# KRLabsOrg/verbatim-rag

Measured on AMD Instinct MI355X. Metric: query x chunk span-extractions/sec @512tok (ModernBERT-base extractor, chunks/s), higher is better.
Workload: dtype bf16

## Files before the change

verbatim-rag_amd/csrc/qkv_attn.hip:

```cpp
#include "host_util.h"
#include "qkv_attn.h"

#include <algorithm>
#include <cstdlib>
#include <type_traits>
#include <vector>

#ifdef VRAG_DEBUG_API
#define VRAG_DBG(bit) ((p.debug_flags & (bit)) != 0)
#else
#define VRAG_DBG(bit) false
#endif

namespace vrag {

constexpr int QA_WB = 192 * 128;
constexpr int QA_XOFF = 2 * QA_WB;
constexpr int QA_TAB = 131072;
constexpr int QA_MU = QA_TAB, QA_RS = QA_TAB + 2048, QA_LS = QA_TAB + 4096;
constexpr int QA_CA = QA_TAB + 5120, QA_SA = QA_CA + 4096, QA_CB = QA_SA + 4096, QA_SB = QA_CB + 2048;
constexpr int QA_SMEM = QA_SB + 2048;
constexpr int QA_V_OFF = 65536;

constexpr float QA_LAZY = 8.0f;
__device__ __forceinline__ float max3f(float a, float b, float c) { return __builtin_fmaxf(__builtin_fmaxf(a, b), c); }

template <int N>
__device__ __forceinline__ void wait_vm() {
  asm volatile("s_waitcnt vmcnt(%0)" ::"n"(N) : "memory");
}

template <bool LOCAL, bool FOLD, typename T>
__global__ __launch_bounds__(512, 2) void qkv_attn_kernel(const QkvAttnParams p) {
  typedef typename Op<T>::v4 V4;
  typedef typename Op<T>::v8 V8;
  extern __shared__ __attribute__((aligned(16))) char smem[];
  const int tid = threadIdx.x;
  const int lane = tid & 63;
  const int wave = uniform(tid >> 6);
  const int g = lane >> 4, l15 = lane & 15;
  const int H = p.H, Tp = p.Tp, nh = p.nh;
  const int xcd = blockIdx.x & 7, slot = blockIdx.x >> 3;
  const int grp = (slot / nh) * 8 + xcd, head = slot % nh;
  if (grp >= p.n_groups) return;
  const int4 wd = p.groups[grp * 8 + wave];
  const int wrow0 = uniform(wd.x), S = uniform(wd.y), kbase = uniform(wd.z);
  const int srow0 = wave * 64;
  const int qrow0 = (wave - kbase) * 64;
  const bool active = qrow0 < S;
  const T* X = reinterpret_cast<const T*>(p.x);
  const T* Wh = reinterpret_cast<const T*>(p.w) + (size_t)head * 192 * H;

  unsigned voffX[2], voffW[3];
#pragma unroll
  for (int par = 0; par < 2; ++par) {
    const int r = par * 8 + (lane >> 3);
    voffX[par] = (unsigned)(r * H + (((lane & 7) ^ ((r >> 1) & 7)) << 3)) * 2u;
  }
#pragma unroll
  for (int i = 0; i < 3; ++i) {
    const int row = wave * 24 + i * 8 + (lane >> 3);
    voffW[i] = (unsigned)(row * H + (((lane & 7) ^ ((row >> 1) & 7)) << 3)) * 2u;
  }
  const char* const Xw = reinterpret_cast<const char*>(X + (size_t)wrow0 * H);
  const char* const Wb = reinterpret_cast<const char*>(Wh);
  char* const xbuf = smem + QA_XOFF + wave * 8192;
  auto dma_w = [&](int kt, int buf, int i) {
    if (VRAG_DBG(4)) return;
    unsigned vo = voffW[i];
    asm volatile("" : "+v"(vo));
    glds16(Wb + kt * 128 + vo, smem + buf * QA_WB + (wave * 24 + i * 8) * 128);
  };
  auto dma_x = [&](int kt, int i) {
    if (!active || VRAG_DBG(4)) return;
    unsigned vo = voffX[i & 1];
    asm volatile("" : "+v"(vo));
    glds16(Xw + ((size_t)(i >> 1) * 16 * H + kt * 64) * 2 + vo, xbuf + i * 1024);
  };

  if (!VRAG_DBG(4)) {
    if (FOLD && lane < 16) {
      glds16(p.ln_mu + min(wrow0 + lane * 4, Tp - 4), smem + QA_MU + srow0 * 4);
      glds16(p.ln_rstd + min(wrow0 + lane * 4, Tp - 4), smem + QA_RS + srow0 * 4);
    }
    if (FOLD && wave == 2) glds16(p.ln_s + head * 192 + lane * 4, smem + QA_LS);
    if (wave == 2 || wave == 3) {
      const float* tab = wave == 2 ? p.rope_cos : p.rope_sin;
#pragma unroll
      for (int i = 0; i < 2; ++i) {
        const int r = i * 8 + (lane >> 3);
        glds16(tab + min(r, p.rope_rows - 1) * 32 + (((lane & 7) ^ ((r >> 1) & 7)) << 2), smem + (wave == 2 ? QA_CB : QA_SB) + i * 1024);
      }
    }
    if (wave == 4 || wave == 5) {
      const float* tab = wave == 4 ? p.rope_cos : p.rope_sin;
#pragma unroll
      for (int i = 0; i < 4; ++i)
        glds16(tab + (size_t)min(16 * (i * 8 + (lane >> 3)), p.rope_rows - 1) * 32 + (lane & 7) * 4, smem + (wave == 4 ? QA_CA : QA_SA) + i * 1024);
    }
  }

  f32x4 acc[12][4];
#pragma unroll
  for (int a = 0; a < 12; ++a)
#pragma unroll
    for (int c = 0; c < 4; ++c) acc[a][c] = f32x4{0.f, 0.f, 0.f, 0.f};

  const int KT = H >> 6;
  int fo[2];
#pragma unroll
  for (int s2 = 0; s2 < 2; ++s2) fo[s2] = l15 * 128 + ((((4 * s2 + g) ^ ((l15 >> 1) & 7))) << 4);
#ifdef VRAG_DEBUG_API
  const int probe = p.debug_flags;
#else
  int probe = 0;
  asm volatile("" : "+s"(probe));
#endif
  const bool mm = active && !(probe & 2);
#pragma unroll
  for (int i = 0; i < 3; ++i) dma_w(0, 0, i);
#pragma unroll
  for (int i = 0; i < 8; ++i) dma_x(0, i);
  for (int kt = 0; kt < KT; ++kt) {
    wait_vm<0>();
    __builtin_amdgcn_s_barrier();
    asm volatile("" ::: "memory");
    const char* sW = smem + (kt & 1) * QA_WB;
    const bool more = kt + 1 < KT;
    V8 xf[2][4], wa;
    if (mm) {
#pragma unroll
      for (int s2 = 0; s2 < 2; ++s2)
#pragma unroll
        for (int rt = 0; rt < 4; ++rt) xf[s2][rt] = *reinterpret_cast<const V8*>(xbuf + rt * 16 * 128 + fo[s2]);
      wa = *reinterpret_cast<const V8*>(sW + fo[0]);
    }
    asm volatile("s_waitcnt lgkmcnt(0)" ::: "memory");
    __builtin_amdgcn_sched_barrier(0);
    if (mm) {
#pragma unroll
      for (int it = 0; it < 24; ++it) {
        const int s2 = it / 12, nj = it % 12;
        V8 na = wa;
        if (it < 23) na = *reinterpret_cast<const V8*>(sW + ((it + 1) % 12) * 16 * 128 + fo[(it + 1) / 12]);
        __builtin_amdgcn_sched_barrier(0);
#pragma unroll
        for (int rt = 0; rt < 4; ++rt) {
          if (nj < 8) acc[nj][rt] = Op<T>::mfma16(wa, xf[s2][rt], acc[nj][rt]);
          else acc[nj][rt] = Op<T>::mfma16(xf[s2][rt], wa, acc[nj][rt]);
        }
        __builtin_amdgcn_sched_barrier(0);
        if (more && it < 11) {
          if (it < 3) dma_w(kt + 1, (kt + 1) & 1, it);
          else dma_x(kt + 1, it - 3);
        }
        __builtin_amdgcn_sched_barrier(0);
        wa = na;
      }
    } else if (more) {
#pragma unroll
      for (int i = 0; i < 3; ++i) dma_w(kt + 1, (kt + 1) & 1, i);
#pragma unroll
      for (int i = 0; i < 8; ++i) dma_x(kt + 1, i);
    }
  }
  __syncthreads();
  if (VRAG_DBG(16)) return;

  const float* l_mu = reinterpret_cast<const float*>(smem + QA_MU) + srow0;
  const float* l_rs = reinterpret_cast<const float*>(smem + QA_RS) + srow0;
  const float* l_ls = reinterpret_cast<const float*>(smem + QA_LS);
#pragma unroll
  for (int db = 0; db < 4; ++db) {
    const int d = db * 16 + l15;
    const float lsv = FOLD ? l_ls[128 + d] : 0.f;
#pragma unroll
    for (int tp = 0; tp < 2; ++tp) {
      V8 vv;
#pragma unroll
      for (int a = 0; a < 2; ++a) {
        const int rt = 2 * tp + a;
        f32x4 m4 = {0.f, 0.f, 0.f, 0.f}, r4 = {1.f, 1.f, 1.f, 1.f};
        if constexpr (FOLD) {
          m4 = *reinterpret_cast<const f32x4*>(l_mu + rt * 16 + 4 * g);
          r4 = *reinterpret_cast<const f32x4*>(l_rs + rt * 16 + 4 * g);
        }
#pragma unroll
        for (int h = 0; h < 2; ++h) {
          const int r0 = 2 * h;
          const f32x2 v = pk_fma(f32x2{-m4[r0], -m4[r0 + 1]}, splat2(lsv), f32x2{acc[8 + db][rt][r0], acc[8 + db][rt][r0 + 1]}) * f32x2{r4[r0], r4[r0 + 1]};
#pragma unroll
          for (int e = 0; e < 2; ++e)
            vv[a * 4 + r0 + e] = qrow0 + rt * 16 + 4 * g + r0 + e < S ? Op<T>::to(v[e], p.f16_sat) : (T)0.f;
        }
      }
      const int c = wave * 8 + tp * 4 + g;
      *reinterpret_cast<V8*>(smem + QA_V_OFF + d * 1024 + ((c ^ l15) << 4)) = vv;
    }
  }
  auto rope_rows = [&](int a0, int rt, int ls_off, float scale, V8 (&out)[2]) {
    const bool live = qrow0 + rt * 16 + l15 < S;
    const float mu = FOLD ? l_mu[rt * 16 + l15] : 0.f, rs = FOLD ? l_rs[rt * 16 + l15] : 1.f;
#pragma unroll
    for (int np = 0; np < 2; ++np) {
      const int dd = np * 16 + 4 * g;
      const f32x4 ca = *reinterpret_cast<const f32x4*>(smem + QA_CA + (((qrow0 >> 4) + rt) * 32 + dd) * 4);
      const f32x4 sa = *reinterpret_cast<const f32x4*>(smem + QA_SA + (((qrow0 >> 4) + rt) * 32 + dd) * 4);
      const int bsw = l15 * 128 + ((((dd >> 2) ^ ((l15 >> 1) & 7))) << 4);
      const f32x4 cb = *reinterpret_cast<const f32x4*>(smem + QA_CB + bsw);
      const f32x4 sb = *reinterpret_cast<const f32x4*>(smem + QA_SB + bsw);
      f32x4 l1 = {0.f, 0.f, 0.f, 0.f}, l2 = {0.f, 0.f, 0.f, 0.f};
      if constexpr (FOLD) {
        l1 = *reinterpret_cast<const f32x4*>(l_ls + ls_off + dd);
        l2 = *reinterpret_cast<const f32x4*>(l_ls + ls_off + 32 + dd);
      }
#pragma unroll
      for (int h = 0; h < 2; ++h) {
        const int j0 = 2 * h;
        f32x2 x1 = {acc[a0 + np][rt][j0], acc[a0 + np][rt][j0 + 1]}, x2 = {acc[a0 + 2 + np][rt][j0], acc[a0 + 2 + np][rt][j0 + 1]};
        if constexpr (FOLD) {
          x1 = pk_fma(splat2(-mu), f32x2{l1[j0], l1[j0 + 1]}, x1) * rs;
          x2 = pk_fma(splat2(-mu), f32x2{l2[j0], l2[j0 + 1]}, x2) * rs;
        }
        const f32x2 ca2 = {ca[j0], ca[j0 + 1]}, sa2 = {sa[j0], sa[j0 + 1]}, cb2 = {cb[j0], cb[j0 + 1]}, sb2 = {sb[j0], sb[j0 + 1]};
        const f32x2 c = pk_fma(-sa2, sb2, ca2 * cb2), sn = pk_fma(ca2, sb2, sa2 * cb2);
        const f32x2 o1 = pk_fma(-x2, sn, x1 * c) * scale, o2 = pk_fma(x1, sn, x2 * c) * scale;
#pragma unroll
        for (int e = 0; e < 2; ++e) {
          if constexpr (!std::is_same<T, bf16_t>::value) {
            out[0][np * 4 + j0 + e] = live ? Op<T>::to(o1[e], p.f16_sat) : (T)0.f;
            out[1][np * 4 + j0 + e] = live ? Op<T>::to(o2[e], p.f16_sat) : (T)0.f;
          } else {
            out[0][np * 4 + j0 + e] = Op<T>::to(o1[e], p.f16_sat);
            out[1][np * 4 + j0 + e] = Op<T>::to(o2[e], p.f16_sat);
          }
        }
      }
    }
  };
#pragma unroll
  for (int rt = 0; rt < 4; ++rt) {
    V8 kf[2];
    rope_rows(4, rt, 64, 1.0f, kf);
    const int row = srow0 + rt * 16 + l15;
#pragma unroll
    for (int s = 0; s < 2; ++s) *reinterpret_cast<V8*>(smem + row * 128 + (((4 * s + g) ^ ((row >> 1) & 7)) << 4)) = kf[s];
  }
  V8 qf[4][2];
#pragma unroll
  for (int rt = 0; rt < 4; ++rt) rope_rows(0, rt, 0, p.q_scale, qf[rt]);
  __syncthreads();

  f32x4 ot[4][4];
  f32x4 lo[4];
#pragma unroll
  for (int c = 0; c < 4; ++c) {
    lo[c] = f32x4{0.f, 0.f, 0.f, 0.f};
#pragma unroll
    for (int dt = 0; dt < 4; ++dt) ot[c][dt] = f32x4{0.f, 0.f, 0.f, 0.f};
  }
  float m_run[4] = {0.f, 0.f, 0.f, 0.f};
  bool seen[4] = {false, false, false, false};
  V8 ones;
#pragma unroll
  for (int j = 0; j < 8; ++j) ones[j] = (T)1.0f;
  const int W = p.window;
  int kt_lo = 0, kt_hi = (S - 1) >> 6;
  if constexpr (LOCAL) {
    kt_lo = max(0, qrow0 - W) >> 6;
    kt_hi = min(S - 1, qrow0 + 63 + W) >> 6;
  }
  const int ksw = (l15 >> 1) & 7;
  if (active && !VRAG_DBG(1)) {
    for (int kt = kt_lo; kt <= kt_hi; ++kt) {
      bool cut[2][2];
#pragma unroll
      for (int u = 0; u < 2; ++u) {
        const int q_lo = qrow0 + 32 * u;
#pragma unroll
        for (int t2 = 0; t2 < 2; ++t2) {
          const int kh = kt * 64 + t2 * 32;
          bool outside = kh >= S || q_lo >= S;
          cut[u][t2] = kh + 31 >= S;
          if constexpr (LOCAL) {
            outside = outside || (kh + 31 < q_lo - W) || (kh > q_lo + 31 + W);
            cut[u][t2] = cut[u][t2] || (kh < q_lo + 31 - W) || (kh + 31 > q_lo + W);
          }
          cut[u][t2] = cut[u][t2] || outside;
        }
      }
      V8 pf[4][2];
      {
        f32x4 st[4][4];
#pragma unroll
        for (int c = 0; c < 4; ++c) {
          const float seed = -m_run[c];
#pragma unroll
          for (int kb = 0; kb < 4; ++kb) st[c][kb] = f32x4{seed, seed, seed, seed};
        }
#pragma unroll
        for (int kb = 0; kb < 4; ++kb) {
          const char* krow = smem + ((kbase + kt) * 64 + kb * 16 + l15) * 128;
          const V8 k0 = *reinterpret_cast<const V8*>(krow + ((g ^ ksw) << 4));
          const V8 k1 = *reinterpret_cast<const V8*>(krow + (((4 + g) ^ ksw) << 4));
#pragma unroll
          for (int c = 0; c < 4; ++c) {
            st[c][kb] = Op<T>::mfma16(k0, qf[c][0], st[c][kb]);
            st[c][kb] = Op<T>::mfma16(k1, qf[c][1], st[c][kb]);
          }
        }
        float mx[4];
#pragma unroll
        for (int c = 0; c < 4; ++c) {
          const int u = c >> 1;
          mx[c] = -INFINITY;
#pragma unroll
          for (int t2 = 0; t2 < 2; ++t2) {
            if (cut[u][t2]) {
              const int qi = qrow0 + 16 * c + l15;
              int lo_k = 0, hi_k = S - 1;
              if constexpr (LOCAL) {
                lo_k = max(0, qi - W);
                hi_k = min(S - 1, qi + W);
              }
              const unsigned span = hi_k >= lo_k ? (unsigned)(hi_k - lo_k) : 0u;
              int d0 = hi_k >= lo_k ? kt * 64 + t2 * 32 + 4 * g - lo_k : -100000;
              asm volatile("" : "+v"(d0));
#pragma unroll
              for (int h2 = 0; h2 < 2; ++h2)
#pragma unroll
                for (int r = 0; r < 4; ++r) {
                  const bool ok = (unsigned)(d0 + 16 * h2 + r) <= span;
                  st[c][2 * t2 + h2][r] = ok ? st[c][2 * t2 + h2][r] : -INFINITY;
                }
            }
            const f32x4& a = st[c][2 * t2];
            const f32x4& b2 = st[c][2 * t2 + 1];
            mx[c] = max3f(mx[c], max3f(a[0], a[1], a[2]), max3f(a[3], b2[0], b2[1]));
            mx[c] = max3f(mx[c], b2[2], b2[3]);
          }
        }
        bool move = false;
#pragma unroll
        for (int c = 0; c < 4; ++c) {
          const bool qlive = qrow0 + 16 * c + l15 < S;
          move = move || (qlive && (mx[c] > QA_LAZY || (!seen[c] && mx[c] > -INFINITY)));
        }
        if (__any(move)) {
#pragma unroll
          for (int c = 0; c < 4; ++c) {
            float m_all = fmaxf(mx[c], __shfl_xor(mx[c], 16, 64));
            m_all = fmaxf(m_all, __shfl_xor(m_all, 32, 64));
            const bool has = m_all > -INFINITY;
            const float delta = seen[c] ? fmaxf(m_all, 0.f) : (has ? m_all : 0.f);
            const float alpha = seen[c] ? __builtin_amdgcn_exp2f(-delta) : 1.0f;
            seen[c] = seen[c] || has;
            m_run[c] += delta;
#pragma unroll
            for (int kb = 0; kb < 4; ++kb)
#pragma unroll
              for (int r = 0; r < 4; ++r) st[c][kb][r] -= delta;
#pragma unroll
            for (int dt = 0; dt < 4; ++dt)
#pragma unroll
              for (int r = 0; r < 4; ++r) ot[c][dt][r] *= alpha;
#pragma unroll
            for (int r = 0; r < 4; ++r) lo[c][r] *= alpha;
          }
        }
#pragma unroll
        for (int c = 0; c < 4; ++c)
#pragma unroll
          for (int t2 = 0; t2 < 2; ++t2)
#pragma unroll
            for (int j = 0; j < 8; ++j) pf[c][t2][j] = (T)__builtin_amdgcn_exp2f(st[c][2 * t2 + (j >> 2)][j & 3]);
      }
#pragma unroll
      for (int t2 = 0; t2 < 2; ++t2) {
#pragma unroll
        for (int c = 0; c < 4; ++c) lo[c] = Op<T>::mfma16(ones, pf[c][t2], lo[c]);
#pragma unroll
        for (int dt = 0; dt < 4; ++dt) {
          const V8 vf = *reinterpret_cast<const V8*>(smem + QA_V_OFF + (dt * 16 + l15) * 1024 + ((((kbase + kt) * 8 + t2 * 4 + g) ^ l15) << 4));
#pragma unroll
          for (int c = 0; c < 4; ++c) ot[c][dt] = Op<T>::mfma16(vf, pf[c][t2], ot[c][dt]);
        }
      }
    }
  }
  __syncthreads();

  if (active) {
    char* stg = smem + wave * 8192;
#pragma unroll
    for (int rt = 0; rt < 4; ++rt) {
      const int row = rt * 16 + l15;
      const bool live = qrow0 + row < S;
      const float inv = live ? 1.0f / lo[rt][0] : 0.f;
#pragma unroll
      for (int db = 0; db < 4; ++db) {
        V4 o;
#pragma unroll
        for (int j = 0; j < 4; ++j) o[j] = live ? Op<T>::to(ot[rt][db][j] * inv, p.f16_sat) : (T)0.f;
        const int c16 = db * 2 + (g >> 1);
        *reinterpret_cast<V4*>(stg + row * 128 + ((c16 ^ (row & 7)) << 4) + ((g & 1) << 3)) = o;
      }
    }
#pragma unroll
    for (int it = 0; it < 8; ++it) {
      const int row = it * 8 + (lane >> 3), c16 = lane & 7;
      const f32x4 v = *reinterpret_cast<const f32x4*>(stg + row * 128 + ((c16 ^ (row & 7)) << 4));
      if (qrow0 + row < S && !VRAG_DBG(8)) store16_nt(reinterpret_cast<T*>(p.o) + (size_t)(wrow0 + row) * H + head * 64 + c16 * 8, v);
    }
  }
}

template <bool LOCAL, bool FOLD, typename T>
static hipError_t launch_t(const QkvAttnParams& p, hipStream_t stream) {
  const hipError_t e = set_max_dynamic_lds<&qkv_attn_kernel<LOCAL, FOLD, T>>(QA_SMEM);
  if (e != hipSuccess) return e;
  const int grid = ((p.n_groups + 7) / 8) * 8 * p.nh;
  hipLaunchKernelGGL((qkv_attn_kernel<LOCAL, FOLD, T>), dim3(grid), dim3(512), QA_SMEM, stream, p);
  return hipGetLastError();
}

hipError_t launch_qkv_attention(const QkvAttnParams& p, bool local, hipStream_t stream) {
  if (p.op_dtype == kOpF16 && !p.f16_sat) return hipErrorInvalidValue;
  if (p.n_groups <= 0) return hipSuccess;
  if (p.H % 64 != 0 || p.H != p.nh * 64 || (size_t)p.Tp * p.H >= (size_t)1 << 31) return hipErrorInvalidValue;
  const bool fold = p.ln_mu != nullptr;
  if (p.op_dtype == kOpF16) {
    if (fold) return local ? launch_t<true, true, f16_t>(p, stream) : launch_t<false, true, f16_t>(p, stream);
    return local ? launch_t<true, false, f16_t>(p, stream) : launch_t<false, false, f16_t>(p, stream);
  }
  if (fold) return local ? launch_t<true, true, bf16_t>(p, stream) : launch_t<false, true, bf16_t>(p, stream);
  return local ? launch_t<true, false, bf16_t>(p, stream) : launch_t<false, false, bf16_t>(p, stream);
}

__global__ void permute_qkv_heads_kernel(const bf16_t* __restrict__ w, const float* __restrict__ s, int H, int nh,
                                         bf16_t* __restrict__ w_out, float* __restrict__ s_out) {
  const int orow = blockIdx.x;
  const int head = orow / 192, part = (orow % 192) / 64, d = orow % 64;
  const int src = part * H + head * 64 + d;
  for (int i = threadIdx.x; i < H; i += blockDim.x) w_out[(size_t)orow * H + i] = w[(size_t)src * H + i];
  if (threadIdx.x == 0 && s && s_out) s_out[orow] = s[src];
}

hipError_t permute_qkv_heads(const bf16_t* w, const float* s, int H, int nh, bf16_t* w_out, float* s_out, hipStream_t stream) {
  hipLaunchKernelGGL(permute_qkv_heads_kernel, dim3(3 * H), dim3(256), 0, stream, w, s, H, nh, w_out, s_out);
  return hipGetLastError();
}

int fused_pack_groups(const int* seq_row, const int* seq_len, int seq0, int seq1, int4* out) {
  int n = 0, used = 8;
  for (int s = seq0; s < seq1; ++s) {
    const int need = (seq_len[s] + 63) / 64;
    if (used + need > 8) {
      for (int w = 0; w < 8; ++w) out[n * 8 + w] = int4{0, 0, 0, 0};
      ++n;
      used = 0;
    }
    for (int j = 0; j < need; ++j) out[(n - 1) * 8 + used + j] = int4{seq_row[s] + 64 * j, seq_len[s], used, 0};
    used += need;
  }
  return n;
}

int pack_groups_best_fit(const int* seq_row, const int* seq_len, int seq0, int seq1, int4* out) {
  std::vector<int> by_need[9];
  for (int s = seq0; s < seq1; ++s) by_need[std::min(8, (seq_len[s] + 63) / 64)].push_back(s);
  std::vector<int> open_with[9];
  std::vector<int> used_of;
  int n = 0;
  for (int need = 8; need >= 1; --need)
    for (int s : by_need[need]) {
      int g = -1;
      for (int room = need; room <= 8 && g < 0; ++room)
        if (!open_with[room].empty()) {
          g = open_with[room].back();
          open_with[room].pop_back();
        }
      if (g < 0) {
        g = n++;
        used_of.push_back(0);
        for (int w = 0; w < 8; ++w) out[g * 8 + w] = int4{0, 0, 0, 0};
      }
      const int used = used_of[g];
      for (int j = 0; j < need; ++j) out[g * 8 + used + j] = int4{seq_row[s] + 64 * j, seq_len[s], used, 0};
      used_of[g] = used + need;
      open_with[8 - used_of[g]].push_back(g);
    }
  return n;
}

}
```

Before: 7739.

## Share RoPE cos/sin between Q and K and skip dead local-window subtiles

The RoPE step now computes the combined cos/sin factors once per row tile and applies them to both K and Q, where before it recomputed them in two separate passes. The attention loop, for local-window layers, also sorts each 32-key half-tile by whether each 32-query half lies fully outside the window. It then skips the QK MFMAs, masking, exp and PV MFMAs for those dead pairs, using compile-time-bounded lambdas so the skipped branches specialise cleanly. The cost is more code and branching, and the dead pf entries are left uninitialised, which relies on every consumer skipping the same pairs.

```diff
diff --git a/verbatim-rag_amd/csrc/qkv_attn.hip b/verbatim-rag_amd/csrc/qkv_attn.hip
--- a/verbatim-rag_amd/csrc/qkv_attn.hip
+++ b/verbatim-rag_amd/csrc/qkv_attn.hip
@@ -198,57 +198,68 @@
       *reinterpret_cast<V8*>(smem + QA_V_OFF + d * 1024 + ((c ^ l15) << 4)) = vv;
     }
   }
-  auto rope_rows = [&](int a0, int rt, int ls_off, float scale, V8 (&out)[2]) {
+  auto rotate = [&](int a0, int rt, int np, int ls_off, float scale, const f32x4& c4, const f32x4& sn4, float mu, float rs, bool live, V8 (&out)[2]) {
+    const int dd = np * 16 + 4 * g;
+    f32x4 l1 = {0.f, 0.f, 0.f, 0.f}, l2 = {0.f, 0.f, 0.f, 0.f};
+    if constexpr (FOLD) {
+      l1 = *reinterpret_cast<const f32x4*>(l_ls + ls_off + dd);
+      l2 = *reinterpret_cast<const f32x4*>(l_ls + ls_off + 32 + dd);
+    }
+#pragma unroll
+    for (int h = 0; h < 2; ++h) {
+      const int j0 = 2 * h;
+      f32x2 x1 = {acc[a0 + np][rt][j0], acc[a0 + np][rt][j0 + 1]}, x2 = {acc[a0 + 2 + np][rt][j0], acc[a0 + 2 + np][rt][j0 + 1]};
+      if constexpr (FOLD) {
+        x1 = pk_fma(splat2(-mu), f32x2{l1[j0], l1[j0 + 1]}, x1) * rs;
+        x2 = pk_fma(splat2(-mu), f32x2{l2[j0], l2[j0 + 1]}, x2) * rs;
+      }
+      const f32x2 c = {c4[j0], c4[j0 + 1]}, sn = {sn4[j0], sn4[j0 + 1]};
+      const f32x2 o1 = pk_fma(-x2, sn, x1 * c) * scale, o2 = pk_fma(x1, sn, x2 * c) * scale;
+#pragma unroll
+      for (int e = 0; e < 2; ++e) {
+        if constexpr (!std::is_same<T, bf16_t>::value) {
+          out[0][np * 4 + j0 + e] = live ? Op<T>::to(o1[e], p.f16_sat) : (T)0.f;
+          out[1][np * 4 + j0 + e] = live ? Op<T>::to(o2[e], p.f16_sat) : (T)0.f;
+        } else {
+          out[0][np * 4 + j0 + e] = Op<T>::to(o1[e], p.f16_sat);
+          out[1][np * 4 + j0 + e] = Op<T>::to(o2[e], p.f16_sat);
+        }
+      }
+    }
+  };
+  V8 qf[4][2];
+#pragma unroll
+  for (int rt = 0; rt < 4; ++rt) {
     const bool live = qrow0 + rt * 16 + l15 < S;
     const float mu = FOLD ? l_mu[rt * 16 + l15] : 0.f, rs = FOLD ? l_rs[rt * 16 + l15] : 1.f;
+    V8 kf[2];
 #pragma unroll
     for (int np = 0; np < 2; ++np) {
+      asm volatile("" ::: "memory");
       const int dd = np * 16 + 4 * g;
       const f32x4 ca = *reinterpret_cast<const f32x4*>(smem + QA_CA + (((qrow0 >> 4) + rt) * 32 + dd) * 4);
       const f32x4 sa = *reinterpret_cast<const f32x4*>(smem + QA_SA + (((qrow0 >> 4) + rt) * 32 + dd) * 4);
       const int bsw = l15 * 128 + ((((dd >> 2) ^ ((l15 >> 1) & 7))) << 4);
       const f32x4 cb = *reinterpret_cast<const f32x4*>(smem + QA_CB + bsw);
       const f32x4 sb = *reinterpret_cast<const f32x4*>(smem + QA_SB + bsw);
-      f32x4 l1 = {0.f, 0.f, 0.f, 0.f}, l2 = {0.f, 0.f, 0.f, 0.f};
-      if constexpr (FOLD) {
-        l1 = *reinterpret_cast<const f32x4*>(l_ls + ls_off + dd);
-        l2 = *reinterpret_cast<const f32x4*>(l_ls + ls_off + 32 + dd);
-      }
+      f32x4 c4, sn4;
 #pragma unroll
       for (int h = 0; h < 2; ++h) {
         const int j0 = 2 * h;
-        f32x2 x1 = {acc[a0 + np][rt][j0], acc[a0 + np][rt][j0 + 1]}, x2 = {acc[a0 + 2 + np][rt][j0], acc[a0 + 2 + np][rt][j0 + 1]};
-        if constexpr (FOLD) {
-          x1 = pk_fma(splat2(-mu), f32x2{l1[j0], l1[j0 + 1]}, x1) * rs;
-          x2 = pk_fma(splat2(-mu), f32x2{l2[j0], l2[j0 + 1]}, x2) * rs;
-        }
         const f32x2 ca2 = {ca[j0], ca[j0 + 1]}, sa2 = {sa[j0], sa[j0 + 1]}, cb2 = {cb[j0], cb[j0 + 1]}, sb2 = {sb[j0], sb[j0 + 1]};
         const f32x2 c = pk_fma(-sa2, sb2, ca2 * cb2), sn = pk_fma(ca2, sb2, sa2 * cb2);
-        const f32x2 o1 = pk_fma(-x2, sn, x1 * c) * scale, o2 = pk_fma(x1, sn, x2 * c) * scale;
-#pragma unroll
-        for (int e = 0; e < 2; ++e) {
-          if constexpr (!std::is_same<T, bf16_t>::value) {
-            out[0][np * 4 + j0 + e] = live ? Op<T>::to(o1[e], p.f16_sat) : (T)0.f;
-            out[1][np * 4 + j0 + e] = live ? Op<T>::to(o2[e], p.f16_sat) : (T)0.f;
-          } else {
-            out[0][np * 4 + j0 + e] = Op<T>::to(o1[e], p.f16_sat);
-            out[1][np * 4 + j0 + e] = Op<T>::to(o2[e], p.f16_sat);
-          }
-        }
-      }
-    }
-  };
-#pragma unroll
-  for (int rt = 0; rt < 4; ++rt) {
-    V8 kf[2];
-    rope_rows(4, rt, 64, 1.0f, kf);
+        c4[j0] = c[0], c4[j0 + 1] = c[1], sn4[j0] = sn[0], sn4[j0 + 1] = sn[1];
+      }
+      rotate(4, rt, np, 64, 1.0f, c4, sn4, mu, rs, live, kf);
+      rotate(0, rt, np, 0, p.q_scale, c4, sn4, mu, rs, live, qf[rt]);
+    }
     const int row = srow0 + rt * 16 + l15;
 #pragma unroll
-    for (int s = 0; s < 2; ++s) *reinterpret_cast<V8*>(smem + row * 128 + (((4 * s + g) ^ ((row >> 1) & 7)) << 4)) = kf[s];
-  }
-  V8 qf[4][2];
-#pragma unroll
-  for (int rt = 0; rt < 4; ++rt) rope_rows(0, rt, 0, p.q_scale, qf[rt]);
+    for (int s = 0; s < 2; ++s) {
+      *reinterpret_cast<V8*>(smem + row * 128 + (((4 * s + g) ^ ((row >> 1) & 7)) << 4)) = kf[s];
+      asm volatile("" : "+v"(qf[rt][s]));
+    }
+  }
   __syncthreads();
 
   f32x4 ot[4][4];
@@ -272,8 +283,9 @@
   }
   const int ksw = (l15 >> 1) & 7;
   if (active && !VRAG_DBG(1)) {
-    for (int kt = kt_lo; kt <= kt_hi; ++kt) {
-      bool cut[2][2];
+    auto attend_tile = [&](const int kt) {
+      constexpr bool PRED = LOCAL;
+      bool cut[2][2], dead[2][2];
 #pragma unroll
       for (int u = 0; u < 2; ++u) {
         const int q_lo = qrow0 + 32 * u;
@@ -286,9 +298,23 @@
             outside = outside || (kh + 31 < q_lo - W) || (kh > q_lo + 31 + W);
             cut[u][t2] = cut[u][t2] || (kh < q_lo + 31 - W) || (kh + 31 > q_lo + W);
           }
+          dead[u][t2] = outside;
           cut[u][t2] = cut[u][t2] || outside;
         }
       }
+      auto for_live = [&](const int t2, auto&& f) {
+        typedef std::integral_constant<int, 0> C0;
+        typedef std::integral_constant<int, 2> C2;
+        typedef std::integral_constant<int, 4> C4;
+        if constexpr (!PRED) {
+          f(C0{}, C4{});
+        } else {
+          const bool a = !dead[0][t2], b = !dead[1][t2];
+          if (a && b) f(C0{}, C4{});
+          else if (a) f(C0{}, C2{});
+          else if (b) f(C2{}, C4{});
+        }
+      };
       V8 pf[4][2];
       {
         f32x4 st[4][4];
@@ -299,16 +325,20 @@
           for (int kb = 0; kb < 4; ++kb) st[c][kb] = f32x4{seed, seed, seed, seed};
         }
 #pragma unroll
-        for (int kb = 0; kb < 4; ++kb) {
-          const char* krow = smem + ((kbase + kt) * 64 + kb * 16 + l15) * 128;
-          const V8 k0 = *reinterpret_cast<const V8*>(krow + ((g ^ ksw) << 4));
-          const V8 k1 = *reinterpret_cast<const V8*>(krow + (((4 + g) ^ ksw) << 4));
-#pragma unroll
-          for (int c = 0; c < 4; ++c) {
-            st[c][kb] = Op<T>::mfma16(k0, qf[c][0], st[c][kb]);
-            st[c][kb] = Op<T>::mfma16(k1, qf[c][1], st[c][kb]);
-          }
-        }
+        for (int t2 = 0; t2 < 2; ++t2)
+          for_live(t2, [&](auto c0, auto c1) {
+#pragma unroll
+            for (int kb = 2 * t2; kb < 2 * t2 + 2; ++kb) {
+              const char* krow = smem + ((kbase + kt) * 64 + kb * 16 + l15) * 128;
+              const V8 k0 = *reinterpret_cast<const V8*>(krow + ((g ^ ksw) << 4));
+              const V8 k1 = *reinterpret_cast<const V8*>(krow + (((4 + g) ^ ksw) << 4));
+#pragma unroll
+              for (int c = decltype(c0)::value; c < decltype(c1)::value; ++c) {
+                st[c][kb] = Op<T>::mfma16(k0, qf[c][0], st[c][kb]);
+                st[c][kb] = Op<T>::mfma16(k1, qf[c][1], st[c][kb]);
+              }
+            }
+          });
         float mx[4];
 #pragma unroll
         for (int c = 0; c < 4; ++c) {
@@ -316,6 +346,7 @@
           mx[c] = -INFINITY;
 #pragma unroll
           for (int t2 = 0; t2 < 2; ++t2) {
+            if (PRED && dead[u][t2]) continue;
             if (cut[u][t2]) {
               const int qi = qrow0 + 16 * c + l15;
               int lo_k = 0, hi_k = S - 1;
@@ -371,22 +402,26 @@
 #pragma unroll
         for (int c = 0; c < 4; ++c)
 #pragma unroll
-          for (int t2 = 0; t2 < 2; ++t2)
+          for (int t2 = 0; t2 < 2; ++t2) {
+            if (PRED && dead[c >> 1][t2]) continue;
 #pragma unroll
             for (int j = 0; j < 8; ++j) pf[c][t2][j] = (T)__builtin_amdgcn_exp2f(st[c][2 * t2 + (j >> 2)][j & 3]);
-      }
-#pragma unroll
-      for (int t2 = 0; t2 < 2; ++t2) {
-#pragma unroll
-        for (int c = 0; c < 4; ++c) lo[c] = Op<T>::mfma16(ones, pf[c][t2], lo[c]);
-#pragma unroll
-        for (int dt = 0; dt < 4; ++dt) {
-          const V8 vf = *reinterpret_cast<const V8*>(smem + QA_V_OFF + (dt * 16 + l15) * 1024 + ((((kbase + kt) * 8 + t2 * 4 + g) ^ l15) << 4));
-#pragma unroll
-          for (int c = 0; c < 4; ++c) ot[c][dt] = Op<T>::mfma16(vf, pf[c][t2], ot[c][dt]);
-        }
-      }
-    }
+          }
+      }
+#pragma unroll
+      for (int t2 = 0; t2 < 2; ++t2)
+        for_live(t2, [&](auto c0, auto c1) {
+#pragma unroll
+          for (int c = decltype(c0)::value; c < decltype(c1)::value; ++c) lo[c] = Op<T>::mfma16(ones, pf[c][t2], lo[c]);
+#pragma unroll
+          for (int dt = 0; dt < 4; ++dt) {
+            const V8 vf = *reinterpret_cast<const V8*>(smem + QA_V_OFF + (dt * 16 + l15) * 1024 + ((((kbase + kt) * 8 + t2 * 4 + g) ^ l15) << 4));
+#pragma unroll
+            for (int c = decltype(c0)::value; c < decltype(c1)::value; ++c) ot[c][dt] = Op<T>::mfma16(vf, pf[c][t2], ot[c][dt]);
+          }
+        });
+    };
+    for (int kt = kt_lo; kt <= kt_hi; ++kt) attend_tile(kt);
   }
   __syncthreads();
 
```

Result: no change. 7764 (median of 5 runs) (+0.3%).
